# cbg-ethz/BnpC

Hardware: AMD Instinct MI355X
Metric: MCMC steps/s, 5k cells x 1k muts (+ cell x cluster log-lik evals/s in ll_evals_per_s_K0) (higher is better)
Workload: dtype f64

## Files before the change

### bnpc_amd/_lib.py

```python
import ctypes as C
import os
import re

import numpy as np

_PKG = os.path.dirname(os.path.abspath(__file__))
LIB_PATH = os.environ.get('BNPC_LIB') or os.path.join(_PKG, 'libbnpc_hip.so')

_environ_raw = getattr(os.environ, '_data', None)
if not isinstance(_environ_raw, dict) \
        or (_environ_raw and not isinstance(next(iter(_environ_raw)), bytes)):
    _environ_raw = None


def env(name, default=None):
    if _environ_raw is None:
        return os.environ.get(name, default)
    val = _environ_raw.get(name.encode() if isinstance(name, str) else name)
    return default if val is None else os.fsdecode(val)


MAX_VIEWS = 7
TILE_SLOTS = 4
MAX_TRIALS = 4
# ... 148 lines not shown
    'bnpc_reload_options': (C.c_int, [_ctx]),
    'bnpc_shape': (C.c_int, [_ctx, _pi64, _pi64]),
    'bnpc_cell_counts': (C.c_int, [_ctx, _pi32, _pi32]),
    'bnpc_view_set': (C.c_int, [_ctx, C.c_int, _pi64, _i64]),
    'bnpc_view_set_slot': (C.c_int, [_ctx, C.c_int, _pi64, _i64, C.c_int]),
    'bnpc_view_size': (C.c_int, [_ctx, C.c_int, _pi64]),
    'bnpc_ll_theta': (C.c_int, [_ctx, C.c_int, _pf, _i64, C.c_double,
        C.c_double, _pd, _i64]),
    'bnpc_ll_theta_pinned': (C.c_int, [_ctx, C.c_int, _pf, _i64, C.c_double,
        C.c_double, _i64, _ppd]),
    'bnpc_ll_theta_pinned_top2': (C.c_int, [_ctx, C.c_int, _pf, _i64,
        C.c_double, C.c_double, _i64, _pd, _ppd, C.POINTER(C.c_void_p)]),
    'bnpc_ll_theta_pinned_top2_issue': (C.c_int, [_ctx, C.c_int, _pf, _i64,
        C.c_double, C.c_double, _i64, _pd, _ppd, C.POINTER(C.c_void_p)]),
    'bnpc_matrix_wait': (C.c_int, [_ctx]),
    'bnpc_hints_wait': (C.c_int, [_ctx]),
    'bnpc_ll_theta_pinned_sums_issue': (C.c_int, [_ctx, C.c_int, _pf, _i64,
        C.c_double, C.c_double, _i64, _pd, _ppd]),
    'bnpc_hints_in_order_issue': (C.c_int, [_ctx, _pi64,
        C.POINTER(C.c_void_p)]),
    'bnpc_theta_put': (C.c_int, [_ctx, _i64, _pf, _i64]),
    'bnpc_ll_rows_pinned': (C.c_int, [_ctx, C.c_int, _pi64, _i64, C.c_double,
        C.c_double, _i64, _ppd]),
    'bnpc_ll_rows_issue': (C.c_int, [_ctx, C.c_int, _pi64, _i64, C.c_double,
        C.c_double, _i64, C.c_int]),
    'bnpc_ll_rows_wait': (C.c_int, [_ctx, C.c_int, _ppd]),
    'bnpc_ll_rows_issue_hint': (C.c_int, [_ctx, C.c_int, _pi64, _i64,
        C.c_double, C.c_double, _i64, C.c_int, _pd]),
    'bnpc_ll_rows_wait_hint': (C.c_int, [_ctx, C.c_int, _ppd,
        C.POINTER(C.c_void_p)]),
    'bnpc_ll_tables': (C.c_int, [_ctx, C.c_int, _pd, _pd, _i64, _pd, _i64]),
    'bnpc_colcounts': (C.c_int, [_ctx, _pi64, _pi64, _i64, _pi32, _pi32]),
    'bnpc_view_counts': (C.c_int, [_ctx, C.c_int, _pi64, _i64, _pi32, _pi32]),
    'bnpc_colcounts_by_label': (C.c_int, [_ctx, _pi64, _pi64, _i64, _pi32,
        _pi32]),
    'bnpc_ll_total': (C.c_int, [_ctx, _pf, _i64, _pd, _pd, C.c_int, _pd]),
    'bnpc_ll_total_issue': (C.c_int, [_ctx, _pf, _i64, _pd, _pd, C.c_int]),
    'bnpc_ll_total_wait': (C.c_int, [_ctx, _pd]),
    'bnpc_bench_ll': (C.c_int, [_ctx, C.c_int, C.POINTER(C.c_float)]),
    'bnpc_bench_ll_full': (C.c_int, [_ctx, C.c_int, C.POINTER(C.c_float)]),
    'bnpc_launch_timers': (C.c_int, [_ctx, C.c_int, C.POINTER(C.c_double),
        C.POINTER(C.c_int64)]),
    'bnpc_mh_ahead_stats': (C.c_int, [_ctx, C.POINTER(C.c_int64),
        C.POINTER(C.c_int64), C.POINTER(C.c_int64)]),
    'bnpc_last_launch': (C.c_int, [_ctx, C.c_char_p, C.c_int,
        C.POINTER(_i64), C.POINTER(C.c_int)]),
    'bnpc_timer_start': (C.c_int, [_ctx]),
    'bnpc_timer_stop': (C.c_int, [_ctx, C.POINTER(C.c_float)]),
    'bnpc_sync': (C.c_int, [_ctx]),
    'bnpc_mt_random_sample': (C.c_double, [C.POINTER(MT19937)]),
    'bnpc_mt_permutation': (C.c_int, [C.POINTER(MT19937), _i64, _pi64]),
    'bnpc_mt_mh_draws': (C.c_int, [C.POINTER(MT19937), _i64, _i64, _i64,
        _pi32, _pd, _pd]),
    'bnpc_mt_beta': (C.c_int, [C.POINTER(MT19937), C.c_void_p, _i64, _pd,
        _pd, _pd]),
    'bnpc_mt_beta_theta': (C.c_int, [C.POINTER(MT19937), C.c_void_p, _i64,
        C.c_double, C.c_double, _pi32, _pi32, C.c_double, C.c_double,
        C.c_double, _pf]),
    'bnpc_log_diff_pi': (C.c_int, [_pd, _pd, _i64, _pd]),
    'bnpc_mh_batch': (C.c_int, [C.c_void_p, C.POINTER(MT19937),
        C.POINTER(MHArgs),
        C.POINTER(C.c_int)]),
    'bnpc_mh_screen': (C.c_int, [_ctx, C.c_int, C.POINTER(MHArgs),
        C.c_void_p, C.c_void_p]),
    'bnpc_mh_batch_dev': (C.c_int, [_ctx, C.c_void_p, C.POINTER(MT19937),
        C.POINTER(MHArgs), C.c_int, C.POINTER(C.c_int)]),
# ... 1320 lines not shown
        n = self.view_size(view)
        if out is None:
            out = np.empty((n, K), dtype=np.float64)
        assert out.flags['C_CONTIGUOUS'] and out.shape[0] == n \
            and out.shape[1] >= K and out.dtype == np.float64
        check(self._lib.bnpc_ll_tables(self._h, view, ptr(L1, C.c_double),
            ptr(L0, C.c_double), K, ptr(out, C.c_double), out.shape[1]),
            'll_tables')
        return out

    def colcounts(self, segments):
        G = len(segments)
        sizes = [len(s) for s in segments]
        offs = np.zeros(G + 1, dtype=np.int64)
        np.cumsum(sizes, out=offs[1:])
        cells = as_i64(np.concatenate([np.asarray(s, dtype=np.int64)
            for s in segments])) if offs[-1] else np.zeros(1, dtype=np.int64)
        n1 = np.zeros((G, self.M), dtype=np.int32)
        n0 = np.zeros((G, self.M), dtype=np.int32)
        check(self._lib.bnpc_colcounts(self._h, ptr(cells, C.c_int64),
            ptr(offs, C.c_int64), G, ptr(n1, C.c_int32), ptr(n0, C.c_int32)),
            'colcounts')
        return n1, n0

    def view_counts(self, view, labels, G):
        labels = as_i64(labels)
        assert labels.size == self.view_size(view)
        n1 = np.empty((G, self.M), dtype=np.int32)
        n0 = np.empty((G, self.M), dtype=np.int32)
        check(self._lib.bnpc_view_counts(self._h, view, ptr(labels, C.c_int64),
            G, ptr(n1, C.c_int32), ptr(n0, C.c_int32)), 'view_counts')
        return n1, n0

    def mh_screen(self, counts_src, old, sd, draws, tmin, tmax, FP, FN, p, q,
                uniform, with_theta=False):
        old = np.ascontiguousarray(old, dtype=np.float32)
        G, M = old.shape
        sd = np.ascontiguousarray(sd, dtype=np.float64)
        sd_idx = np.ascontiguousarray(draws[0], dtype=np.int32)
        U = np.ascontiguousarray(draws[1], dtype=np.float64)
        u = np.ascontiguousarray(draws[2], dtype=np.float64)
        a = MHArgs()
        a.G, a.M = G, M
        a.old_theta, a.sd, a.n_sd = ptr(old), ptr(sd), sd.size
        a.tmin, a.tmax, a.FP, a.FN, a.p, a.q = tmin, tmax, FP, FN, p, q
        a.uniform_prior, a.trans_prob = int(bool(uniform)), 0
        a.sd_idx, a.U, a.u = ptr(sd_idx), ptr(U), ptr(u)
        flags = np.empty((G, M), dtype=np.uint8)
        new32 = np.full((G, M), np.nan, dtype=np.float32)
        check(self._lib.bnpc_mh_screen(self._h, counts_src, C.byref(a),
            ptr(flags), ptr(new32)), 'mh_screen')
        return (flags, new32) if with_theta else flags

    def mh_screen_stats(self):
        seen, kept = _i64(0), _i64(0)
        check(self._lib.bnpc_mh_screen_stats(self._h, C.byref(seen),
            C.byref(kept)), 'mh_screen_stats')
        return seen.value, kept.value

    def reload_options(self):
        check(self._lib.bnpc_reload_options(self._h), 'reload_options')

    def colcounts_by_label(self, assignment, ids, fetch=True):
        assignment = as_i64(assignment)
        ids = as_i64(ids)
        K = ids.size
# ... 80 lines not shown
```

### bnpc_amd/csrc/bnpc_context.cpp

```cpp

#include <hip/hip_runtime.h>
#include <atomic>
#include <stdarg.h>
#include <stdint.h>
#include <stdio.h>
#include <stdlib.h>
#include <string.h>
#include <sys/mman.h>
#include <mutex>
#include <vector>
#include <algorithm>

#include "bnpc_ctx.h"

static thread_local char g_err[512] = "";

void bnpc_set_error(const char *fmt, ...)
{
    va_list ap;
    va_start(ap, fmt);
    vsnprintf(g_err, sizeof(g_err), fmt, ap);
    va_end(ap);
}

// ... 135 lines not shown
{
    if (c->total_pending) HIPCHK(hipStreamSynchronize(c->stream));
    c->stage_used = 0;
    return 0;
}

int wait_done(bnpc_ctx *c, int slot, unsigned seq)
{
    if (seq) {
        const volatile unsigned *f = c->done_pin + 16 * slot;
        for (int spins = 0; spins < 20000; spins++) {
            if ((int)(*f - seq) >= 0) {
                std::atomic_thread_fence(std::memory_order_acquire);
                return 0;
            }
            bnpc_cpu_relax();
        }
    }
    HIPCHK(hipStreamSynchronize(c->stream));
    return 0;
}

const void *stage_in_place(bnpc_ctx *c, const void *src, size_t bytes)
{
    if (!c->tun.zero_copy || (int64_t)bytes > ZC_IN_MAX) return nullptr;
    void *slot = stage_slot(c, bytes);
    if (!slot || !c->stage_dev) return nullptr;
    memcpy(slot, src, bytes);
    return c->stage_dev + ((char *)slot - (char *)c->stage);
}

void *zc_result(bnpc_ctx *c, size_t bytes, void **dev)
{
    if (!c->tun.zero_copy || (int64_t)bytes > ZC_OUT_MAX
        || bytes > ZC_OUT_BYTES)
        return nullptr;
    if (!c->zc_out) {
        if (hipHostMalloc(&c->zc_out, ZC_OUT_BYTES, hipHostMallocDefault)
                != hipSuccess) {
            c->zc_out = nullptr;
            return nullptr;
        }
        void *d = nullptr;
        if (hipHostGetDevicePointer(&d, c->zc_out, 0) != hipSuccess) {
            (void)hipHostFree(c->zc_out);
            c->zc_out = nullptr;
            return nullptr;
        }
        c->zc_out_dev = (char *)d;
    }
    *dev = c->zc_out_dev;
    return c->zc_out;
}

int h2d(bnpc_ctx *c, void *dst, const void *src, size_t bytes)
{
    void *slot = stage_slot(c, bytes);
    if (slot) {
        memcpy(slot, src, bytes);
        src = slot;
    }
    HIPCHK(hipMemcpyAsync(dst, src, bytes, hipMemcpyHostToDevice, c->stream));
    return 0;
}

int d2h_begin(bnpc_ctx *c, D2H &t, void *dst, const void *src,
              size_t bytes)
{
// ... 380 lines not shown
```

### bnpc_amd/csrc/bnpc_ctx.h

```cpp
#ifndef BNPC_CTX_H
#define BNPC_CTX_H
#include <hip/hip_runtime.h>
#include <stdint.h>
#include <string.h>
#include <algorithm>
#include <vector>

#include "bnpc_hip.h"
#include "bnpc_internal.h"

#define HIPCHK(expr)                                                         \
    do {                                                                     \
        hipError_t e_ = (expr);                                              \
        if (e_ != hipSuccess) {                                              \
            bnpc_set_error("%s failed: %s (%s:%d)", #expr,                   \
                           hipGetErrorString(e_), __FILE__, __LINE__);       \
            return 1;                                                        \
        }                                                                    \
    } while (0)

#define ARGCHK(cond, msg)                                                    \
    do {                                                                     \
        if (!(cond)) {                                                       \
            bnpc_set_error("bad argument: %s", msg);                         \
// ... 221 lines not shown
    explicit SideLane(bnpc_ctx *ctx)
        : c(ctx), on(ctx->side_stream && ctx->any_tile_pending())
    {
        if (on) flip();
    }
    ~SideLane()
    {
        if (on) flip();
    }
    void flip()
    {
        std::swap(c->stream, c->side_stream);
        std::swap(c->theta, c->side_theta);
        std::swap(c->tabs, c->side_tabs);
        std::swap(c->out, c->side_out);
        std::swap(c->part, c->side_part);
    }
};

struct MHPin {
    double *U, *u;
    int32_t *sd_idx;
    float *theta;
    float *new32;
    uint8_t *flags;
};

#pragma GCC visibility push(hidden)
void *stage_slot(bnpc_ctx *c, size_t bytes);
int arena_reset(bnpc_ctx *c);
int wait_done(bnpc_ctx *c, int slot, unsigned seq);
const void *stage_in_place(bnpc_ctx *c, const void *src, size_t bytes);
void *zc_result(bnpc_ctx *c, size_t bytes, void **dev);
int h2d(bnpc_ctx *c, void *dst, const void *src, size_t bytes);
int d2h_begin(bnpc_ctx *c, D2H &t, void *dst, const void *src, size_t bytes);
void d2h_finish(const D2H &t);
int ensure_pin(bnpc_ctx *c, size_t bytes);
int ensure_host(void **p, size_t *cap, size_t bytes);
int ensure_lanes(bnpc_ctx *c);
int build_view(bnpc_ctx *c, int view, const long long *d_cells, int64_t n);
int colcounts_by_label_impl(bnpc_ctx *c, const int64_t *assignment,
                            const int64_t *ids, int64_t K, int32_t *n1,
                            int32_t *n0, const int **defer);
int view_label_counts(bnpc_ctx *c, int view, const int64_t *labels,
                      int64_t G, int32_t *n1, int32_t *n0,
                      const int **defer);
int mh_screen_launch(bnpc_ctx *c, int src, const bnpc_mh_args *a,
                     const MHPin &dev, int64_t g0 = 0, int64_t Gp = -1,
                     DoneSignal sig = {nullptr, nullptr, 0},
                     int64_t row0 = 0, int64_t G_all = -1);
void mh_ahead_destroy(bnpc_ctx *c);
#pragma GCC visibility pop

#endif
```

### bnpc_amd/csrc/bnpc_internal.h

```cpp
#ifndef BNPC_INTERNAL_H
#define BNPC_INTERNAL_H
#include <math.h>
#include <stdarg.h>
#include <stdint.h>

#include "bnpc_hip.h"

void bnpc_set_error(const char *fmt, ...);

#ifdef __cplusplus
#include <linux/futex.h>
#include <stdlib.h>
#include <sys/syscall.h>
#include <time.h>
#include <unistd.h>

#include <atomic>
#include <functional>
#include <thread>

static inline void bnpc_cpu_relax()
{
#if defined(__x86_64__)
    __builtin_ia32_pause();
// ... 59 lines not shown

const unsigned long long *bnpc_ctx_row(const bnpc_ctx *c, int64_t cell,
                                       int64_t *M, int *W);
void bnpc_legacy_beta_row(bnpc_mt19937 *rng, bnpc_legacy_gauss *g, int64_t M,
                          const unsigned long long *row, double p, double q,
                          double tmin, double tmax, float *theta);

uint64_t bnpc_ctx_label_counts_generation(const bnpc_ctx *c);
int bnpc_sweep_open_cluster(bnpc_gibbs_state *st, bnpc_mt19937 *rng,
                            int64_t cell, double *ll, int64_t *assignment,
                            int64_t *col_of_id, int64_t *col_id,
                            int64_t *col_size, int64_t *order);
double bnpc_legacy_gamma(bnpc_mt19937 *rng, bnpc_legacy_gauss *g, double shape,
                         double scale);

void bnpc_mh_rank0_hook(const std::function<void()> *hook);
void bnpc_mh_row_gate(const std::function<bool(int64_t)> *gate);
#ifdef __cplusplus
int bnpc_mh_ahead_begin(bnpc_ctx *c, const bnpc_mt19937 *rng,
                        const bnpc_legacy_gauss *g,
                        const std::function<bool(bnpc_mt19937 *,
                                                 bnpc_legacy_gauss *)> &prelude,
                        int64_t rows, int64_t M, int64_t n_sd, bool *posted,
                        int64_t min_entries = -1);
void bnpc_mh_ahead_drop(bnpc_ctx *c);
void bnpc_mh_ahead_scan(bnpc_ctx *c, const bnpc_mt19937 *rng, int64_t uniforms,
                        int64_t rows, int64_t M, int64_t n_sd);
void bnpc_rg_scan_order_hook(const std::function<void()> *hook);
void bnpc_move_last_draw_hook(const std::function<void(int)> *hook);
#endif
int bnpc_ll_theta_begin(bnpc_ctx *c, int view, const float *theta, int64_t K,
                        double FP, double FN, double *out, int64_t ldo);
int bnpc_ll_theta_end(bnpc_ctx *c);
int bnpc_rg_scan_step_with(bnpc_ctx *ctx, const bnpc_host_kernels *k,
                           bnpc_mt19937 *rng, int view, int64_t n,
                           int64_t *rg_assignment, double DP_a,
                           const bnpc_mh_args *mh, int32_t *n1, int32_t *n0,
                           double *scan_log_prob, int *status,
                           const double *ll_ready);
int bnpc_rg_counts_and_batch(bnpc_ctx *c, const bnpc_host_kernels *k,
                             bnpc_mt19937 *rng, int view,
                             const int64_t *labels, const bnpc_mh_args *a,
                             int32_t *n1, int32_t *n0, int *status);

#ifdef __cplusplus
void mt_refill_block(uint32_t *key);
#endif
static inline void mt_refill(bnpc_mt19937 *s)
{
    mt_refill_block(s->key);
    s->pos = 0;
}

static inline uint32_t mt_next32(bnpc_mt19937 *s)
{
    if (s->pos >= 624) mt_refill(s);
    uint32_t y = s->key[s->pos++];
    y ^= (y >> 11);
    y ^= (y << 7) & 0x9d2c5680u;
    y ^= (y << 15) & 0xefc60000u;
    y ^= (y >> 18);
    return y;
}

static inline double mt_double(bnpc_mt19937 *s)
{
// ... 115 lines not shown
```

### bnpc_amd/csrc/bnpc_kernels.hip

```cpp

#include <hip/hip_runtime.h>
#include <hip/hip_ext.h>
#include <stdint.h>
#include <stdio.h>
#include <stdlib.h>
#include <string.h>
#include <math.h>
#include <vector>
#include <algorithm>

#include "bnpc_ctx.h"

struct LaunchTimers {
    bool on = false;
    std::vector<hipEvent_t> ev;
    size_t used = 0;
    hipEvent_t *next_pair()
    {
        if (used + 2 > ev.size()) {
            const size_t old = ev.size();
            ev.resize(old + 512, nullptr);
            for (size_t i = old; i < ev.size(); i++)
                if (hipEventCreate(&ev[i]) != hipSuccess) {
                    ev.resize(i & ~(size_t)1);
// ... 980 lines not shown
#pragma unroll
            for (int j = 0; j < CM_SEG; j++) {
                c1[j] += __popcll(mk.x & mem[j]);
                c0[j] += __popcll(mk.y & mem[j]);
            }
        }
    }
    __syncthreads();
    int (*red)[2 * CM_SEG][64] = (int (*)[2 * CM_SEG][64])mem_lds;
#pragma unroll
    for (int j = 0; j < CM_SEG; j++) {
        red[wave][2 * j][lane] = c1[j];
        red[wave][2 * j + 1][lane] = c0[j];
    }
    __syncthreads();
#pragma unroll
    for (int i = 0; i < CM_SEG / 4; i++) {
        const int j = wave + 4 * i;
        if (g0 + j < G && m < M) {
            const int s1 = red[0][2 * j][lane] + red[1][2 * j][lane]
                + red[2][2 * j][lane] + red[3][2 * j][lane];
            const int s0 = red[0][2 * j + 1][lane] + red[1][2 * j + 1][lane]
                + red[2][2 * j + 1][lane] + red[3][2 * j + 1][lane];
            const size_t at = (size_t)(g0 + j) * M + m;
            n1[at] = s1;
            n0[at] = s0;
            if (h1) {
                h1[at] = s1;
                h0[at] = s0;
            }
        }
    }
    signal_done(done);
}

#define TOTAL_BLOCKS 256

__global__ __launch_bounds__(256) void k_ll_total(
    const float *__restrict__ theta, const int *__restrict__ n1,
    const int *__restrict__ n0, long long KM, int E, double FP0, double FN0,
    double FP1, double FN1, double FP2, double FN2, double FP3, double FN3,
    double *__restrict__ partial, DoneSignal done)
{
    const double FPs[4] = {FP0, FP1, FP2, FP3};
    const double FNs[4] = {FN0, FN1, FN2, FN3};
    double acc[4] = {0.0, 0.0, 0.0, 0.0};
    const long long stride = (long long)gridDim.x * 256;
    for (long long i = (long long)blockIdx.x * 256 + threadIdx.x; i < KM;
         i += stride) {
        const int c1 = n1[i], c0 = n0[i];
        if ((c1 | c0) == 0) continue;
        const float th = theta[i];
        const double th64 = (double)th;
        const double om64 = (double)(1.0f - th);
#pragma unroll
        for (int e = 0; e < 4; e++) {
            if (e < E) {
                const double l1 = log(th64 * (1.0 - FNs[e]) + om64 * FPs[e]);
                const double l0 = log(th64 * FNs[e] + om64 * (1.0 - FPs[e]));
                acc[e] += (double)c1 * l1 + (double)c0 * l0;
            }
        }
    }
    __shared__ double red[4][256];
#pragma unroll
    for (int e = 0; e < 4; e++) red[e][threadIdx.x] = acc[e];
// ... 938 lines not shown
                                       const int64_t *rows, int64_t K,
                                       double FP, double FN, int64_t ldo,
                                       int slot, const double *col_prior)
{
    ARGCHK(col_prior, "col_prior is NULL");
    return ll_rows_issue_impl(c, view, rows, K, FP, FN, ldo, slot, col_prior);
}

extern "C" int bnpc_ll_rows_wait_hint(bnpc_ctx *c, int slot, double **host,
                                      bnpc_top2 **hint)
{
    ARGCHK(hint, "NULL argument");
    *hint = nullptr;
    const bool hinted = c && slot >= 0 && slot < BNPC_TILE_SLOTS
        && c->tile_hinted[slot];
    if (int rc = bnpc_ll_rows_wait(c, slot, host)) return rc;
    if (hinted) *hint = (bnpc_top2 *)c->tile_hint[slot];
    return 0;
}

extern "C" int bnpc_ll_rows_wait(bnpc_ctx *c, int slot, double **host)
{
    ARGCHK(c && host, "NULL argument");
    ARGCHK(slot >= 0 && slot < BNPC_TILE_SLOTS, "slot out of range");
    *host = nullptr;
    ARGCHK(c->tile_pending[slot], "no tile was issued on this slot");
    HIPCHK(hipSetDevice(c->device));
    c->tile_pending[slot] = false;
    HIPCHK(hipEventSynchronize(c->tile_done[slot]));
    *host = (double *)c->tile_pin[slot];
    return 0;
}

extern "C" int bnpc_ll_tables(bnpc_ctx *c, int view, const double *L1,
                              const double *L0, int64_t K, double *out,
                              int64_t ldo)
{
    ARGCHK(c, "ctx is NULL");
    ARGCHK(view >= 0 && view < BNPC_MAX_VIEWS, "view out of range");
    ARGCHK(K >= 0 && (K == 0 || (L1 && L0)), "table is NULL");
    HIPCHK(hipSetDevice(c->device));
    if (K == 0) return 0;
    const size_t bytes = (size_t)K * c->M * sizeof(double);
    if (arena_reset(c)) return 1;
    c->tab_src = nullptr;
    if (c->tun.zero_copy && (int64_t)(2 * bytes) <= ZC_IN_MAX) {
        void *slot = stage_slot(c, 2 * bytes);
        if (slot && c->stage_dev) {
            memcpy(slot, L1, bytes);
            memcpy((char *)slot + bytes, L0, bytes);
            c->tab_src = (const double *)(c->stage_dev
                + ((char *)slot - (char *)c->stage));
        }
    }
    if (!c->tab_src) {
        if (ensure(c->tab_in, 2 * bytes)) return 1;
        if (h2d(c, c->tab_in.p, L1, bytes)) return 1;
        if (h2d(c, (char *)c->tab_in.p + bytes, L0, bytes)) return 1;
        c->tab_src = (const double *)c->tab_in.p;
    }
    int rc = ll_common(c, view, K, ldo, false, 0.0, 0.0, out);
    if (!out && rc == 0) HIPCHK(hipStreamSynchronize(c->stream));
    return rc;
}

static int colcounts_device(bnpc_ctx *c, const int64_t *cells, int64_t n_cells,
                            const int64_t *seg_offsets, int64_t G,
                            DevBuf &cnt)
{
    if (arena_reset(c)) return 1;
    const size_t cnt_bytes = (size_t)2 * G * c->M * sizeof(int32_t);
    if (ensure(cnt, cnt_bytes)) return 1;
    HIPCHK(hipMemsetAsync(cnt.p, 0, cnt_bytes, c->stream));
    std::vector<Chunk> chunks;
    const int64_t CH = 32;
    for (int64_t g = 0; g < G; g++)
        for (int64_t b = seg_offsets[g]; b < seg_offsets[g + 1]; b += CH)
            chunks.push_back(
                {(long long)b,
                 (long long)std::min<int64_t>(seg_offsets[g + 1], b + CH),
                 (long long)g});
    if (chunks.empty()) return 0;
    if (ensure(c->cells, n_cells * sizeof(long long))) return 1;
    if (ensure(c->chunks, chunks.size() * sizeof(Chunk))) return 1;
    if (h2d(c, c->cells.p, cells, n_cells * sizeof(long long))) return 1;
    if (h2d(c, c->chunks.p, chunks.data(), chunks.size() * sizeof(Chunk)))
        return 1;
    int *n1 = (int *)cnt.p;
    int *n0 = n1 + (size_t)G * c->M;
    const size_t maxy = 65535;
    for (size_t off = 0; off < chunks.size(); off += maxy) {
        const size_t ny = std::min(maxy, chunks.size() - off);
        dim3 grid((unsigned)((c->M + 255) / 256), (unsigned)ny);
        BNPC_LAUNCH(k_colcounts, grid, dim3(256), 0, c->stream,
                           c->rows, c->W, (int)c->M,
                           (const long long *)c->cells.p,
                           (const Chunk *)c->chunks.p + off, n1, n0);
        HIPCHK(hipGetLastError());
    }
    HIPCHK(hipStreamSynchronize(c->stream));
    return 0;
}

template <typename LabelOf>
static int counts_from_masks(bnpc_ctx *c, int view, LabelOf label_of,
                             int64_t G, DevBuf &cnt, int32_t *n1, int32_t *n0,
                             const int **defer = nullptr)
{
    if (defer) *defer = nullptr;
    const View &v = c->views[view];
    const size_t half = (size_t)G * c->M * sizeof(int32_t);
    if (ensure(cnt, 2 * half)) return 1;
    if (arena_reset(c)) return 1;
    if (v.n == 0) {
        HIPCHK(hipMemsetAsync(cnt.p, 0, 2 * half, c->stream));
        HIPCHK(hipStreamSynchronize(c->stream));
        if (n1) memset(n1, 0, half);
        if (n0) memset(n0, 0, half);
        return 0;
    }
    const size_t mem_bytes = (size_t)G * v.nblk * sizeof(unsigned long long);
    unsigned long long *mem = nullptr;
    const unsigned long long *d_mem = nullptr;
    std::vector<unsigned long long> heap;
    if (c->tun.zero_copy && (int64_t)mem_bytes <= ZC_IN_MAX) {
        mem = (unsigned long long *)stage_slot(c, mem_bytes);
        if (mem && c->stage_dev)
            d_mem = (const unsigned long long *)(c->stage_dev
                + ((char *)mem - (char *)c->stage));
        else
            mem = nullptr;
    }
    if (!mem) {
        heap.resize((size_t)G * v.nblk);
        mem = heap.data();
    }
    memset(mem, 0, mem_bytes);
    for (int64_t s = 0; s < v.n; s++) {
        const int64_t g = label_of(s);
        if (g >= G) {
            bnpc_set_error("bad argument: segment label out of range");
            return 2;
        }
        if (g >= 0) mem[(size_t)g * v.nblk + (s >> 6)] |= 1ull << (s & 63);
    }
    if (!d_mem) {
        if (ensure(c->chunks, mem_bytes)) return 1;
        HIPCHK(hipMemcpyAsync(c->chunks.p, mem, mem_bytes,
                              hipMemcpyHostToDevice, c->stream));
        d_mem = (const unsigned long long *)c->chunks.p;
    }
    void *zc_dev = nullptr;
    int *zc_host = (n1 && n0) ? (int *)zc_result(c, 2 * half, &zc_dev)
                              : nullptr;
    int *d1 = (int *)cnt.p, *d0 = d1 + (size_t)G * c->M;
    int *h1 = zc_host ? (int *)zc_dev : nullptr;
    int *h0 = h1 ? h1 + (size_t)G * c->M : nullptr;
    dim3 grid((unsigned)(c->Mpad / 64), (unsigned)((G + CM_SEG - 1) / CM_SEG));
    const long long range = std::min<long long>(v.nblk, CM_RANGE_MAX);
    size_t lds = (size_t)range * CM_SEG * sizeof(unsigned long long);
    const size_t red_bytes = 4 * 2 * CM_SEG * 64 * sizeof(int);
    if (lds < red_bytes) lds = red_bytes;
    unsigned done_seq = 0;
    const DoneSignal sig = (zc_host && !defer) ? make_signal(c, 0, &done_seq)
                                               : DoneSignal{nullptr, nullptr, 0};
    BNPC_LAUNCH(k_counts_masks, grid, dim3(256), lds, c->stream,
                       (const ulonglong2 *)v.masks.p, c->Mpad, (int)c->M,
                       (long long)v.nblk, d_mem, (int)G, d1, d0, h1, h0,
                       range, sig);
    HIPCHK(hipGetLastError());
    if (zc_host && defer) {
        *defer = zc_host;
    } else if (zc_host) {
        if (int rc = wait_done(c, 0, done_seq)) return rc;
        memcpy(n1, zc_host, half);
        memcpy(n0, zc_host + (size_t)G * c->M, half);
    } else if (n1 && n0) {
        void *slot = stage_slot(c, 2 * half);
        if (slot) {
            HIPCHK(hipMemcpyAsync(slot, cnt.p, 2 * half,
                                  hipMemcpyDeviceToHost, c->stream));
            HIPCHK(hipStreamSynchronize(c->stream));
            memcpy(n1, slot, half);
            memcpy(n0, (char *)slot + half, half);
        } else {
            HIPCHK(hipMemcpyAsync(n1, d1, half, hipMemcpyDeviceToHost,
                                  c->stream));
            HIPCHK(hipMemcpyAsync(n0, d0, half, hipMemcpyDeviceToHost,
                                  c->stream));
            HIPCHK(hipStreamSynchronize(c->stream));
        }
    } else {
        HIPCHK(hipStreamSynchronize(c->stream));
    }
    return 0;
}

extern "C" int bnpc_view_counts(bnpc_ctx *c, int view, const int64_t *labels,
                                int64_t G, int32_t *n1, int32_t *n0)
{
    ARGCHK(c && n1 && n0, "NULL argument");
    ARGCHK(view >= 0 && view < BNPC_MAX_VIEWS, "view out of range");
    ARGCHK(G > 0 && G <= 4096, "G out of range");
    ARGCHK(c->views[view].n == 0 || labels, "labels is NULL");
    HIPCHK(hipSetDevice(c->device));
    SideLane lane(c);
    c->cnt_rows = 0;
    int rc = counts_from_masks(c, view,
        [=](int64_t s) -> int64_t { return labels[s]; }, G, c->cnt, n1, n0);
    if (rc == 0) c->cnt_rows = G;
    return rc;
}

int view_label_counts(bnpc_ctx *c, int view, const int64_t *labels,
                      int64_t G, int32_t *n1, int32_t *n0, const int **defer)
{
    return counts_from_masks(c, view,
        [=](int64_t s) -> int64_t { return labels[s]; }, G, c->cnt, n1, n0,
        defer);
}

extern "C" int bnpc_colcounts(bnpc_ctx *c, const int64_t *cells,
                              const int64_t *seg_offsets, int64_t G,
                              int32_t *n1, int32_t *n0)
{
    ARGCHK(c && seg_offsets && n1 && n0, "NULL argument");
    ARGCHK(G >= 0, "G negative");
    if (G == 0) return 0;
    ARGCHK(seg_offsets[0] == 0, "seg_offsets[0] must be 0");
    const int64_t n = seg_offsets[G];
    for (int64_t g = 0; g < G; g++)
        ARGCHK(seg_offsets[g] <= seg_offsets[g + 1], "seg_offsets not sorted");
    ARGCHK(n == 0 || cells, "cells is NULL");
    for (int64_t i = 0; i < n; i++)
        ARGCHK(cells[i] >= 0 && cells[i] < c->N, "cell index out of range");
    HIPCHK(hipSetDevice(c->device));
    c->cnt_rows = 0;
    if (colcounts_device(c, cells, n, seg_offsets, G, c->cnt)) return 1;
    const size_t half = (size_t)G * c->M * sizeof(int32_t);
    D2H a, b;
    if (d2h_begin(c, a, n1, c->cnt.p, half)) return 1;
    if (d2h_begin(c, b, n0, (char *)c->cnt.p + half, half)) return 1;
    HIPCHK(hipStreamSynchronize(c->stream));
    d2h_finish(a);
    d2h_finish(b);
    return 0;
}

int colcounts_by_label_impl(bnpc_ctx *c, const int64_t *assignment,
                            const int64_t *ids, int64_t K,
                            int32_t *n1, int32_t *n0,
                            const int **defer)
// ... 329 lines not shown
```

### bnpc_amd/csrc/bnpc_moves.cpp

```cpp
#include <stdio.h>
#include <stdlib.h>
#include <time.h>
#include <algorithm>
#include <cstring>
#include <vector>

#include "bnpc_internal.h"

namespace {

struct Scratch {
    std::vector<int64_t> cells, others, rg, labels, perm, target;
    std::vector<double> probs, cdf, work, L, ll, ll_first, tmp, U, u, A, std2;
    std::vector<int32_t> n1, n0, sd_idx;
    std::vector<float> rows, fresh, gather;
};

struct Restore {
    bnpc_mt19937 *rng;
    bnpc_legacy_gauss *g;
    bnpc_mt19937 rng0;
    bnpc_legacy_gauss g0;
    bool armed;
    Restore(bnpc_mt19937 *r, bnpc_legacy_gauss *gg)
// ... 244 lines not shown
    const int64_t *cells = s.cells.data();
    st->n_cells = n;
    mark();

    int rc = bnpc_view_set(ctx, st->view, cells, n);
    if (rc) return rc;
    {
        int W = 0;
        int64_t Mr = 0;
        const unsigned long long *row[2] = {
            bnpc_ctx_row(ctx, cells[0], &Mr, &W),
            bnpc_ctx_row(ctx, cells[n - 1], &Mr, &W)};
        if (!row[0] || !row[1] || Mr != M) return 0;
        const double vals[3] = {1.0, 0.0, st->fill};
        double arg[6], lg[6];
        for (int v = 0; v < 3; v++) {
            const double t = vals[v], om = 1 - vals[v];
            arg[v] = t * (1 - FN) + om * FP;
            arg[3 + v] = t * FN + om * (1 - FP);
        }
        np_loop(k->np_log, k->np_log_data, arg, lg, 6);
        s.L.resize((size_t)4 * M);
        for (int r = 0; r < 2; r++) {
            for (int64_t m = 0; m < M; m++) {
                const unsigned long long bit = 1ull << (m & 63);
                const int v = (row[r][2 * (m >> 6)] & bit) ? 0
                    : (row[r][2 * (m >> 6) + 1] & bit) ? 1 : 2;
                s.L[(size_t)r * M + m] = lg[v];
                s.L[(size_t)(2 + r) * M + m] = lg[3 + v];
            }
        }
    }
    s.ll.resize((size_t)n * 2);
    rc = bnpc_ll_tables(ctx, st->view, s.L.data(), s.L.data() + 2 * M, 2,
                        s.ll.data(), 0);
    if (rc) return rc;
    s.rg.resize((size_t)S);
    s.labels.resize((size_t)n);
    for (int64_t t = 0; t < S; t++)
        s.rg[t] = s.ll[2 * (t + 1) + 1] > s.ll[2 * (t + 1)] ? 1 : 0;
    auto set_labels = [&]() {
        s.labels[0] = 0;
        for (int64_t t = 0; t < S; t++) s.labels[t + 1] = s.rg[t] ? 1 : 0;
        s.labels[n - 1] = 1;
    };
    set_labels();
    mark();
    s.n1.resize((size_t)3 * M);
    s.n0.resize((size_t)3 * M);
    int32_t *n1 = s.n1.data(), *n0 = s.n0.data();
    rc = bnpc_view_counts(ctx, st->view, s.labels.data(), 2, n1, n0);
    if (rc) return rc;
    auto sum_rows = [&]() {
        for (int64_t m = 0; m < M; m++) {
            n1[2 * M + m] = n1[m] + n1[M + m];
            n0[2 * M + m] = n0[m] + n0[M + m];
        }
    };
    sum_rows();
    mark();
    s.rows.resize((size_t)3 * M);
    s.fresh.resize((size_t)3 * M);
    float *rows = s.rows.data(), *fresh = s.fresh.data();
    const bool ahead = st->scan_no > 0 || split;
    bool begun = false;
    for (int g = 0; g < 3; g++) {
        if (g == 2 && ahead) {
            s.ll_first.resize((size_t)n * 2);
            rc = bnpc_ll_theta_begin(ctx, st->view, rows, 2, FP, FN,
                                     s.ll_first.data(), 0);
            if (rc) return rc;
            begun = true;
        }
        rc = bnpc_mt_beta_theta(rng, gauss, M, st->p, st->q, n1 + g * M,
                                n0 + g * M, 1.0, st->tmin, st->tmax,
                                rows + g * M);
        if (rc) {
            if (begun) (void)bnpc_ll_theta_end(ctx);
            return rc;
        }
    }
    if (begun) {
        rc = bnpc_ll_theta_end(ctx);
        if (rc) return rc;
    }
// ... 200 lines not shown
        if (last_draw) (*last_draw)(1);
        s.std2.resize((size_t)2 * M);
        for (int64_t m = 0; m < 2 * M; m++) s.std2[m] = st->sd[s.sd_idx[m]];
        memcpy(s.gather.data(), st->parameters + cl_i * st->param_stride,
               (size_t)M * sizeof(float));
        memcpy(s.gather.data() + M, st->parameters + cl_j * st->param_stride,
               (size_t)M * sizeof(float));
        double prob2[2] = {0, 0};
        bnpc_accept_args la;
        memset(&la, 0, sizeof la);
        la.G = 2;
        la.M = M;
        la.new_theta = s.gather.data();
        la.old_theta = rows;
        la.std = s.std2.data();
        la.n1 = n1;
        la.n0 = n0;
        la.fmin = 0.0;
        la.fmax = 1.0;
        la.tmin = st->tmin;
        la.tmax = st->tmax;
        la.FP = FP;
        la.FN = FN;
        la.p = st->p;
        la.q = st->q;
        la.uniform_prior = st->uniform_prior;
        la.clip = 1;
        la.A = s.A.data();
        la.sum = prob2;
        la.threads = st->threads_wide;
        rc = bnpc_log_accept(k, &la, &sub);
        if (rc) return rc;
        if (sub) return 0;
        rc = bnpc_ll_theta(ctx, st->view, s.gather.data(), 2, FP, FN,
                           s.ll.data(), 0);
        if (rc) return rc;
        s.target.resize((size_t)S);
        for (int64_t t = 0; t < S; t++)
            s.target[t] = st->assignment[cells[t + 1]] == cl_i ? 0 : 1;
        double prob_assign = 0.0;
        rc = bnpc_rg_scan(nullptr, 1, S, s.ll.data() + 2, st->DP_a,
                          s.rg.data(), s.target.data(), &prob_assign);
        if (rc) return rc;
        const double gs_split = prob2[0] + prob2[1] + prob_assign;
        const double trans = gs_split - gs_merge;
        mark();

        const int64_t n_j = rg_ones() + 1, n_i = n - n_j;
        double lprior = k->gammaln((double)n, 0) - log_a;
        if (n_i > 0) lprior -= k->gammaln((double)n_i, 0);
        if (n_j > 0) lprior -= k->gammaln((double)n_j, 0);
        if (!st->uniform_prior) {
            double sum_merged = 0.0, sum_own = 0.0;
            s.work.resize((size_t)2 * M);
            rc = bnpc_beta_logpdf_f32(k, merged, M, st->p, st->q, nullptr,
                                      nullptr, s.work.data(), &sum_merged,
                                      st->threads_wide);
            if (rc) return rc;
            rc = bnpc_beta_logpdf_f32(k, s.gather.data(), 2 * M, st->p, st->q,
                                      nullptr, nullptr, s.work.data(),
                                      &sum_own, st->threads_wide);
            if (rc) return rc;
            lprior += sum_merged - sum_own;
        }
        mark();
        set_labels();
        rc = bnpc_view_counts(ctx, st->view, s.labels.data(), 2, n1, n0);
        if (rc) return rc;
        const double ll_i = subset_ll_sum(k, rows, n1, n0, nullptr, nullptr,
                                          M, FP, FN, s);
        const double ll_j = subset_ll_sum(k, rows + M, n1 + M, n0 + M,
                                          nullptr, nullptr, M, FP, FN, s);
        const double ll_all = subset_ll_sum(k, merged, n1, n0, n1 + M, n0 + M,
                                            M, FP, FN, s);
        const double llr = ll_all - ll_i - ll_j;
        mark();
        if (S - 1 <= 0) return 0;
        const double rev = -np_log1(k, (double)N) - np_log1(k, (double)(S - 1));
        const double size_ratio = rev - size_data;
        A = trans + lprior + llr + size_ratio;
        if (np_log1(k, mt_double(rng)) < A) {
            memcpy(st->parameters + cl_i * st->param_stride, merged,
                   (size_t)M * sizeof(float));
            for (int64_t t = n_first; t < n; t++)
                st->assignment[cells[t]] = cl_i;
            st->accepted = 1;
            st->cl_i = cl_i;
            st->cl_j = cl_j;
            st->moved = n - n_first;
        }
    }
    st->log_A = A;
    restore.armed = false;
    *status = 0;
    report(split ? "split" : "merge");
    return 0;
}
```

### include/bnpc_hip.h

```cpp
#ifndef BNPC_HIP_H
#define BNPC_HIP_H

#include <stdint.h>

#ifdef __cplusplus
extern "C" {
#endif

typedef struct bnpc_ctx bnpc_ctx;

#define BNPC_MAX_VIEWS 7
#define BNPC_TILE_SLOTS 4
#define BNPC_MAX_TRIALS 4

const char *bnpc_last_error(void);
int bnpc_abi_version(void);
int bnpc_device_count(int *count);
int bnpc_device_info(int device, char *name, int len, int *cus);

int bnpc_device_pci_bus_id(int device, char *bus_id, int len);

int bnpc_team_stress(int64_t jobs, int max_tasks, int ranks, uint64_t seed,
                     int64_t *done, int64_t *expected);
int bnpc_team_size(int threads);
// ... 50 lines not shown
                                    bnpc_top2 **top2);
int bnpc_hints_wait(bnpc_ctx *ctx);
int bnpc_ll_theta_pinned_sums_issue(bnpc_ctx *ctx, int view,
                                    const float *theta, int64_t K, double FP,
                                    double FN, int64_t ldo,
                                    const double *col_prior, double **host);
int bnpc_hints_in_order_issue(bnpc_ctx *ctx, const int64_t *order,
                              bnpc_top2 **top2);
int bnpc_matrix_wait(bnpc_ctx *ctx);

int bnpc_theta_put(bnpc_ctx *ctx, int64_t row0, const float *theta, int64_t R);
int bnpc_ll_rows_pinned(bnpc_ctx *ctx, int view, const int64_t *rows,
                        int64_t K, double FP, double FN, int64_t ldo,
                        double **host);

int bnpc_ll_rows_issue(bnpc_ctx *ctx, int view, const int64_t *rows, int64_t K,
                       double FP, double FN, int64_t ldo, int slot);
int bnpc_ll_rows_wait(bnpc_ctx *ctx, int slot, double **host);
int bnpc_ll_rows_issue_hint(bnpc_ctx *ctx, int view, const int64_t *rows,
                            int64_t K, double FP, double FN, int64_t ldo,
                            int slot, const double *col_prior);
int bnpc_ll_rows_wait_hint(bnpc_ctx *ctx, int slot, double **host,
                           bnpc_top2 **hint);

int bnpc_ll_tables(bnpc_ctx *ctx, int view, const double *L1, const double *L0,
                   int64_t K, double *out, int64_t ldo);

int bnpc_colcounts(bnpc_ctx *ctx, const int64_t *cells,
                   const int64_t *seg_offsets, int64_t G,
                   int32_t *n1, int32_t *n0);

int bnpc_view_counts(bnpc_ctx *ctx, int view, const int64_t *labels,
                     int64_t G, int32_t *n1, int32_t *n0);

int bnpc_colcounts_by_label(bnpc_ctx *ctx, const int64_t *assignment,
                            const int64_t *ids, int64_t K,
                            int32_t *n1, int32_t *n0);

int bnpc_ll_total(bnpc_ctx *ctx, const float *theta, int64_t K,
                  const double *FP, const double *FN, int E, double *out);
int bnpc_ll_total_issue(bnpc_ctx *ctx, const float *theta, int64_t K,
                        const double *FP, const double *FN, int E);
int bnpc_ll_total_wait(bnpc_ctx *ctx, double *out);

int bnpc_bench_ll(bnpc_ctx *ctx, int reps, float *ms_per_launch);
int bnpc_bench_ll_full(bnpc_ctx *ctx, int reps, float *ms_per_call);
int bnpc_last_launch(const bnpc_ctx *ctx, char *name, int len, int64_t *K,
                     int *mutation_chunks);
int bnpc_mh_ahead_stats(bnpc_ctx *ctx, int64_t *begun, int64_t *taken,
                        int64_t *rows);
int bnpc_launch_timers(bnpc_ctx *ctx, int on, double *device_ms,
                       int64_t *launches);
int bnpc_timer_start(bnpc_ctx *ctx);
int bnpc_timer_stop(bnpc_ctx *ctx, float *ms);
int bnpc_sync(bnpc_ctx *ctx);

typedef struct bnpc_mt19937 {
    uint32_t key[624];
    int32_t pos;
} bnpc_mt19937;

double bnpc_mt_random_sample(bnpc_mt19937 *rng);
int bnpc_mt_permutation(bnpc_mt19937 *rng, int64_t n, int64_t *out);

int bnpc_mt_mh_draws(bnpc_mt19937 *rng, int64_t G, int64_t M, int64_t n_sd,
                     int32_t *sd_idx, double *U, double *u);
// ... 306 lines not shown
```

Before: 2939.

## Fuse launch-state label derivation and column counts on device; overlap merge counts

In the split-merge move, launch-state log-likelihoods and the per-group column counts are now produced in one device sequence. A new ballot kernel builds membership masks straight from the likelihood output, so the host no longer round-trips to derive labels before launching the count kernel. In the merge path, the count kernel is queued behind the theta log-likelihood launch and its results land at an offset in the zero-copy buffer, so the two overlap instead of running as separate synchronous calls. This adds offset management in the shared zero-copy buffer and more complex deferred-completion handling.

```diff
diff --git a/bnpc_amd/_lib.py b/bnpc_amd/_lib.py
--- a/bnpc_amd/_lib.py
+++ b/bnpc_amd/_lib.py
@@ -204,6 +204,8 @@
     'bnpc_ll_tables': (C.c_int, [_ctx, C.c_int, _pd, _pd, _i64, _pd, _i64]),
     'bnpc_colcounts': (C.c_int, [_ctx, _pi64, _pi64, _i64, _pi32, _pi32]),
     'bnpc_view_counts': (C.c_int, [_ctx, C.c_int, _pi64, _i64, _pi32, _pi32]),
+    'bnpc_ll_tables_counts': (C.c_int, [_ctx, C.c_int, _pd, _pd, _pd, _pi32,
+        _pi32]),
     'bnpc_colcounts_by_label': (C.c_int, [_ctx, _pi64, _pi64, _i64, _pi32,
         _pi32]),
     'bnpc_ll_total': (C.c_int, [_ctx, _pf, _i64, _pd, _pd, C.c_int, _pd]),
@@ -1590,6 +1592,18 @@
             G, ptr(n1, C.c_int32), ptr(n0, C.c_int32)), 'view_counts')
         return n1, n0
 
+    def ll_tables_counts(self, view, L1, L0):
+        L1 = np.ascontiguousarray(L1, dtype=np.float64)
+        L0 = np.ascontiguousarray(L0, dtype=np.float64)
+        assert L1.shape == L0.shape == (2, self.M)
+        ll = np.empty((self.view_size(view), 2), dtype=np.float64)
+        n1 = np.empty((2, self.M), dtype=np.int32)
+        n0 = np.empty((2, self.M), dtype=np.int32)
+        check(self._lib.bnpc_ll_tables_counts(self._h, view,
+            ptr(L1, C.c_double), ptr(L0, C.c_double), ptr(ll, C.c_double),
+            ptr(n1, C.c_int32), ptr(n0, C.c_int32)), 'll_tables_counts')
+        return ll, n1, n0
+
     def mh_screen(self, counts_src, old, sd, draws, tmin, tmax, FP, FN, p, q,
                 uniform, with_theta=False):
         old = np.ascontiguousarray(old, dtype=np.float32)
diff --git a/bnpc_amd/csrc/bnpc_context.cpp b/bnpc_amd/csrc/bnpc_context.cpp
--- a/bnpc_amd/csrc/bnpc_context.cpp
+++ b/bnpc_amd/csrc/bnpc_context.cpp
@@ -191,8 +191,13 @@
 
 void *zc_result(bnpc_ctx *c, size_t bytes, void **dev)
 {
+    return zc_result_at(c, 0, bytes, dev);
+}
+
+void *zc_result_at(bnpc_ctx *c, size_t at, size_t bytes, void **dev)
+{
     if (!c->tun.zero_copy || (int64_t)bytes > ZC_OUT_MAX
-        || bytes > ZC_OUT_BYTES)
+        || at + bytes > ZC_OUT_BYTES)
         return nullptr;
     if (!c->zc_out) {
         if (hipHostMalloc(&c->zc_out, ZC_OUT_BYTES, hipHostMallocDefault)
diff --git a/bnpc_amd/csrc/bnpc_ctx.h b/bnpc_amd/csrc/bnpc_ctx.h
--- a/bnpc_amd/csrc/bnpc_ctx.h
+++ b/bnpc_amd/csrc/bnpc_ctx.h
@@ -277,6 +277,7 @@
 int wait_done(bnpc_ctx *c, int slot, unsigned seq);
 const void *stage_in_place(bnpc_ctx *c, const void *src, size_t bytes);
 void *zc_result(bnpc_ctx *c, size_t bytes, void **dev);
+void *zc_result_at(bnpc_ctx *c, size_t at, size_t bytes, void **dev);
 int h2d(bnpc_ctx *c, void *dst, const void *src, size_t bytes);
 int d2h_begin(bnpc_ctx *c, D2H &t, void *dst, const void *src, size_t bytes);
 void d2h_finish(const D2H &t);
diff --git a/bnpc_amd/csrc/bnpc_internal.h b/bnpc_amd/csrc/bnpc_internal.h
--- a/bnpc_amd/csrc/bnpc_internal.h
+++ b/bnpc_amd/csrc/bnpc_internal.h
@@ -115,6 +115,8 @@
 int bnpc_ll_theta_begin(bnpc_ctx *c, int view, const float *theta, int64_t K,
                         double FP, double FN, double *out, int64_t ldo);
 int bnpc_ll_theta_end(bnpc_ctx *c);
+int bnpc_view_counts_behind(bnpc_ctx *c, int view, const int64_t *labels,
+                            int32_t *n1, int32_t *n0);
 int bnpc_rg_scan_step_with(bnpc_ctx *ctx, const bnpc_host_kernels *k,
                            bnpc_mt19937 *rng, int view, int64_t n,
                            int64_t *rg_assignment, double DP_a,
diff --git a/bnpc_amd/csrc/bnpc_kernels.hip b/bnpc_amd/csrc/bnpc_kernels.hip
--- a/bnpc_amd/csrc/bnpc_kernels.hip
+++ b/bnpc_amd/csrc/bnpc_kernels.hip
@@ -1036,6 +1036,27 @@
         }
     }
     signal_done(done);
+}
+
+__global__ __launch_bounds__(64) void k_launch_members(
+    const double *__restrict__ ll, long long ldo, long long n, long long nblk,
+    unsigned long long *__restrict__ member)
+{
+    const long long blk = blockIdx.x;
+    const long long s = blk * 64 + threadIdx.x;
+    const bool in = s < n;
+    bool one = false;
+    if (in) {
+        one = ll[(size_t)s * ldo + 1] > ll[(size_t)s * ldo];
+        if (s == 0) one = false;
+        if (s == n - 1) one = true;
+    }
+    const unsigned long long w0 = __ballot(in && !one);
+    const unsigned long long w1 = __ballot(in && one);
+    if (threadIdx.x == 0) {
+        member[blk] = w0;
+        member[nblk + blk] = w1;
+    }
 }
 
 #define TOTAL_BLOCKS 256
@@ -2040,15 +2061,9 @@
     return 0;
 }
 
-extern "C" int bnpc_ll_tables(bnpc_ctx *c, int view, const double *L1,
-                              const double *L0, int64_t K, double *out,
-                              int64_t ldo)
-{
-    ARGCHK(c, "ctx is NULL");
-    ARGCHK(view >= 0 && view < BNPC_MAX_VIEWS, "view out of range");
-    ARGCHK(K >= 0 && (K == 0 || (L1 && L0)), "table is NULL");
-    HIPCHK(hipSetDevice(c->device));
-    if (K == 0) return 0;
+static int stage_tables(bnpc_ctx *c, const double *L1, const double *L0,
+                        int64_t K)
+{
     const size_t bytes = (size_t)K * c->M * sizeof(double);
     if (arena_reset(c)) return 1;
     c->tab_src = nullptr;
@@ -2067,6 +2082,19 @@
         if (h2d(c, (char *)c->tab_in.p + bytes, L0, bytes)) return 1;
         c->tab_src = (const double *)c->tab_in.p;
     }
+    return 0;
+}
+
+extern "C" int bnpc_ll_tables(bnpc_ctx *c, int view, const double *L1,
+                              const double *L0, int64_t K, double *out,
+                              int64_t ldo)
+{
+    ARGCHK(c, "ctx is NULL");
+    ARGCHK(view >= 0 && view < BNPC_MAX_VIEWS, "view out of range");
+    ARGCHK(K >= 0 && (K == 0 || (L1 && L0)), "table is NULL");
+    HIPCHK(hipSetDevice(c->device));
+    if (K == 0) return 0;
+    if (int rc = stage_tables(c, L1, L0, K)) return rc;
     int rc = ll_common(c, view, K, ldo, false, 0.0, 0.0, out);
     if (!out && rc == 0) HIPCHK(hipStreamSynchronize(c->stream));
     return rc;
@@ -2110,16 +2138,41 @@
     return 0;
 }
 
+static int counts_launch(bnpc_ctx *c, const View &v,
+                         const unsigned long long *d_mem, int64_t G,
+                         DevBuf &cnt, int *h1, DoneSignal sig)
+{
+    int *d1 = (int *)cnt.p, *d0 = d1 + (size_t)G * c->M;
+    int *h0 = h1 ? h1 + (size_t)G * c->M : nullptr;
+    dim3 grid((unsigned)(c->Mpad / 64), (unsigned)((G + CM_SEG - 1) / CM_SEG));
+    const long long range = std::min<long long>(v.nblk, CM_RANGE_MAX);
+    size_t lds = (size_t)range * CM_SEG * sizeof(unsigned long long);
+    const size_t red_bytes = 4 * 2 * CM_SEG * 64 * sizeof(int);
+    if (lds < red_bytes) lds = red_bytes;
+    BNPC_LAUNCH(k_counts_masks, grid, dim3(256), lds, c->stream,
+                       (const ulonglong2 *)v.masks.p, c->Mpad, (int)c->M,
+                       (long long)v.nblk, d_mem, (int)G, d1, d0, h1, h0,
+                       range, sig);
+    HIPCHK(hipGetLastError());
+    return 0;
+}
+
+struct CountsBehind {
+    size_t zc_at;
+    unsigned seq;
+};
+
 template <typename LabelOf>
 static int counts_from_masks(bnpc_ctx *c, int view, LabelOf label_of,
                              int64_t G, DevBuf &cnt, int32_t *n1, int32_t *n0,
-                             const int **defer = nullptr)
+                             const int **defer = nullptr,
+                             CountsBehind *behind = nullptr)
 {
     if (defer) *defer = nullptr;
     const View &v = c->views[view];
     const size_t half = (size_t)G * c->M * sizeof(int32_t);
     if (ensure(cnt, 2 * half)) return 1;
-    if (arena_reset(c)) return 1;
+    if (!behind && arena_reset(c)) return 1;
     if (v.n == 0) {
         HIPCHK(hipMemsetAsync(cnt.p, 0, 2 * half, c->stream));
         HIPCHK(hipStreamSynchronize(c->stream));
@@ -2158,25 +2211,18 @@
                               hipMemcpyHostToDevice, c->stream));
         d_mem = (const unsigned long long *)c->chunks.p;
     }
+    const size_t zc_at = behind ? (behind->zc_at + 255) & ~(size_t)255 : 0;
     void *zc_dev = nullptr;
-    int *zc_host = (n1 && n0) ? (int *)zc_result(c, 2 * half, &zc_dev)
-                              : nullptr;
+    int *zc_host = (n1 && n0)
+        ? (int *)zc_result_at(c, zc_at, 2 * half, &zc_dev) : nullptr;
+    if (zc_host) zc_host = (int *)((char *)zc_host + zc_at);
     int *d1 = (int *)cnt.p, *d0 = d1 + (size_t)G * c->M;
-    int *h1 = zc_host ? (int *)zc_dev : nullptr;
-    int *h0 = h1 ? h1 + (size_t)G * c->M : nullptr;
-    dim3 grid((unsigned)(c->Mpad / 64), (unsigned)((G + CM_SEG - 1) / CM_SEG));
-    const long long range = std::min<long long>(v.nblk, CM_RANGE_MAX);
-    size_t lds = (size_t)range * CM_SEG * sizeof(unsigned long long);
-    const size_t red_bytes = 4 * 2 * CM_SEG * 64 * sizeof(int);
-    if (lds < red_bytes) lds = red_bytes;
+    int *h1 = zc_host ? (int *)((char *)zc_dev + zc_at) : nullptr;
     unsigned done_seq = 0;
-    const DoneSignal sig = (zc_host && !defer) ? make_signal(c, 0, &done_seq)
-                                               : DoneSignal{nullptr, nullptr, 0};
-    BNPC_LAUNCH(k_counts_masks, grid, dim3(256), lds, c->stream,
-                       (const ulonglong2 *)v.masks.p, c->Mpad, (int)c->M,
-                       (long long)v.nblk, d_mem, (int)G, d1, d0, h1, h0,
-                       range, sig);
-    HIPCHK(hipGetLastError());
+    const DoneSignal sig = (zc_host && (!defer || behind))
+        ? make_signal(c, 0, &done_seq) : DoneSignal{nullptr, nullptr, 0};
+    if (behind) behind->seq = done_seq;
+    if (int rc = counts_launch(c, v, d_mem, G, cnt, h1, sig)) return rc;
     if (zc_host && defer) {
         *defer = zc_host;
     } else if (zc_host) {
@@ -2226,6 +2272,97 @@
     return counts_from_masks(c, view,
         [=](int64_t s) -> int64_t { return labels[s]; }, G, c->cnt, n1, n0,
         defer);
+}
+
+int bnpc_view_counts_behind(bnpc_ctx *c, int view, const int64_t *labels,
+                            int32_t *n1, int32_t *n0)
+{
+    ARGCHK(c && n1 && n0 && labels, "NULL argument");
+    ARGCHK(view >= 0 && view < BNPC_MAX_VIEWS, "view out of range");
+    if (!c->defer_set || c->views[view].n == 0)
+        return bnpc_view_counts(c, view, labels, 2, n1, n0);
+    HIPCHK(hipSetDevice(c->device));
+    c->cnt_rows = 0;
+    const int *pending = nullptr;
+    CountsBehind behind = {c->defer.bytes, 0};
+    int rc = counts_from_masks(c, view,
+        [=](int64_t s) -> int64_t { return labels[s]; }, 2, c->cnt, n1, n0,
+        &pending, &behind);
+    if (rc) {
+        (void)hipStreamSynchronize(c->stream);
+        return rc;
+    }
+    c->cnt_rows = 2;
+    if (!pending) return 0;
+    if (int rw = wait_done(c, 0, behind.seq)) return rw;
+    const size_t half = (size_t)2 * c->M * sizeof(int32_t);
+    memcpy(n1, pending, half);
+    memcpy(n0, pending + (size_t)2 * c->M, half);
+    return 0;
+}
+
+extern "C" int bnpc_ll_tables_counts(bnpc_ctx *c, int view, const double *L1,
+                                     const double *L0, double *ll,
+                                     int32_t *n1, int32_t *n0)
+{
+    ARGCHK(c && L1 && L0 && ll && n1 && n0, "NULL argument");
+    ARGCHK(view >= 0 && view < BNPC_MAX_VIEWS, "view out of range");
+    HIPCHK(hipSetDevice(c->device));
+    const View &v = c->views[view];
+    const int64_t n = v.n;
+    ARGCHK(n >= 2, "a launch state has two anchors");
+    if (int rc = stage_tables(c, L1, L0, 2)) return rc;
+    c->defer_set = false;
+    c->defer_next = !c->any_tile_pending();
+    int rc = ll_common(c, view, 2, 2, false, 0.0, 0.0, ll);
+    c->defer_next = false;
+    if (rc) {
+        c->defer_set = false;
+        return rc;
+    }
+    const size_t half = (size_t)2 * c->M * sizeof(int32_t);
+    void *zc_dev = nullptr;
+    const size_t zc_at = (c->defer.bytes + 255) & ~(size_t)255;
+    int *zc_host = c->defer_set
+        ? (int *)zc_result_at(c, zc_at, 2 * half, &zc_dev) : nullptr;
+    if (!zc_host) {
+        if (int re = bnpc_ll_theta_end(c)) return re;
+        std::vector<int64_t> labels((size_t)n);
+        for (int64_t s = 0; s < n; s++)
+            labels[(size_t)s] = ll[2 * s + 1] > ll[2 * s] ? 1 : 0;
+        labels[0] = 0;
+        labels[(size_t)n - 1] = 1;
+        return bnpc_view_counts(c, view, labels.data(), 2, n1, n0);
+    }
+    auto fail = [&](int code) {
+        (void)hipStreamSynchronize(c->stream);
+        c->defer_set = false;
+        return code;
+    };
+    c->cnt_rows = 0;
+    const size_t mem_bytes = (size_t)2 * v.nblk * sizeof(unsigned long long);
+    if (ensure(c->chunks, mem_bytes) || ensure(c->cnt, 2 * half))
+        return fail(1);
+    BNPC_LAUNCH(k_launch_members, dim3((unsigned)v.nblk), dim3(64), 0,
+                       c->stream, (const double *)c->last_out, 2ll,
+                       (long long)n, (long long)v.nblk,
+                       (unsigned long long *)c->chunks.p);
+    if (hipGetLastError() != hipSuccess) {
+        bnpc_set_error("k_launch_members could not be launched");
+        return fail(1);
+    }
+    unsigned done_seq = 0;
+    const DoneSignal sig = make_signal(c, 0, &done_seq);
+    if (counts_launch(c, v, (const unsigned long long *)c->chunks.p, 2, c->cnt,
+                      (int *)((char *)zc_dev + zc_at), sig))
+        return fail(1);
+    c->cnt_rows = 2;
+    if (int rw = wait_done(c, 0, done_seq)) return fail(rw);
+    if (int re = bnpc_ll_theta_end(c)) return re;
+    zc_host = (int *)((char *)zc_host + zc_at);
+    memcpy(n1, zc_host, half);
+    memcpy(n0, zc_host + (size_t)2 * c->M, half);
+    return 0;
 }
 
 extern "C" int bnpc_colcounts(bnpc_ctx *c, const int64_t *cells,
diff --git a/bnpc_amd/csrc/bnpc_moves.cpp b/bnpc_amd/csrc/bnpc_moves.cpp
--- a/bnpc_amd/csrc/bnpc_moves.cpp
+++ b/bnpc_amd/csrc/bnpc_moves.cpp
@@ -300,25 +300,16 @@
         }
     }
     s.ll.resize((size_t)n * 2);
-    rc = bnpc_ll_tables(ctx, st->view, s.L.data(), s.L.data() + 2 * M, 2,
-                        s.ll.data(), 0);
-    if (rc) return rc;
-    s.rg.resize((size_t)S);
-    s.labels.resize((size_t)n);
-    for (int64_t t = 0; t < S; t++)
-        s.rg[t] = s.ll[2 * (t + 1) + 1] > s.ll[2 * (t + 1)] ? 1 : 0;
-    auto set_labels = [&]() {
-        s.labels[0] = 0;
-        for (int64_t t = 0; t < S; t++) s.labels[t + 1] = s.rg[t] ? 1 : 0;
-        s.labels[n - 1] = 1;
-    };
-    set_labels();
-    mark();
     s.n1.resize((size_t)3 * M);
     s.n0.resize((size_t)3 * M);
     int32_t *n1 = s.n1.data(), *n0 = s.n0.data();
-    rc = bnpc_view_counts(ctx, st->view, s.labels.data(), 2, n1, n0);
+    rc = bnpc_ll_tables_counts(ctx, st->view, s.L.data(), s.L.data() + 2 * M,
+                               s.ll.data(), n1, n0);
     if (rc) return rc;
+    mark();
+    s.rg.resize((size_t)S);
+    for (int64_t t = 0; t < S; t++)
+        s.rg[t] = s.ll[2 * (t + 1) + 1] > s.ll[2 * (t + 1)] ? 1 : 0;
     auto sum_rows = [&]() {
         for (int64_t m = 0; m < M; m++) {
             n1[2 * M + m] = n1[m] + n1[M + m];
@@ -585,12 +576,23 @@
         rc = bnpc_log_accept(k, &la, &sub);
         if (rc) return rc;
         if (sub) return 0;
-        rc = bnpc_ll_theta(ctx, st->view, s.gather.data(), 2, FP, FN,
-                           s.ll.data(), 0);
-        if (rc) return rc;
         s.target.resize((size_t)S);
         for (int64_t t = 0; t < S; t++)
             s.target[t] = st->assignment[cells[t + 1]] == cl_i ? 0 : 1;
+        s.labels.resize((size_t)n);
+        s.labels[0] = 0;
+        for (int64_t t = 0; t < S; t++) s.labels[t + 1] = s.target[t];
+        s.labels[n - 1] = 1;
+        rc = bnpc_ll_theta_begin(ctx, st->view, s.gather.data(), 2, FP, FN,
+                                 s.ll.data(), 0);
+        if (rc) return rc;
+        rc = bnpc_view_counts_behind(ctx, st->view, s.labels.data(), n1, n0);
+        if (rc) {
+            (void)bnpc_ll_theta_end(ctx);
+            return rc;
+        }
+        rc = bnpc_ll_theta_end(ctx);
+        if (rc) return rc;
         double prob_assign = 0.0;
         rc = bnpc_rg_scan(nullptr, 1, S, s.ll.data() + 2, st->DP_a,
                           s.rg.data(), s.target.data(), &prob_assign);
@@ -617,9 +619,6 @@
             lprior += sum_merged - sum_own;
         }
         mark();
-        set_labels();
-        rc = bnpc_view_counts(ctx, st->view, s.labels.data(), 2, n1, n0);
-        if (rc) return rc;
         const double ll_i = subset_ll_sum(k, rows, n1, n0, nullptr, nullptr,
                                           M, FP, FN, s);
         const double ll_j = subset_ll_sum(k, rows + M, n1 + M, n0 + M,
diff --git a/include/bnpc_hip.h b/include/bnpc_hip.h
--- a/include/bnpc_hip.h
+++ b/include/bnpc_hip.h
@@ -106,6 +106,10 @@
 
 int bnpc_view_counts(bnpc_ctx *ctx, int view, const int64_t *labels,
                      int64_t G, int32_t *n1, int32_t *n0);
+
+int bnpc_ll_tables_counts(bnpc_ctx *ctx, int view, const double *L1,
+                          const double *L0, double *ll, int32_t *n1,
+                          int32_t *n0);
 
 int bnpc_colcounts_by_label(bnpc_ctx *ctx, const int64_t *assignment,
                             const int64_t *ids, int64_t K,
```

Result: slower. 2434 (-17.2%).
